# openhumanoids/pronto

Measured on AMD Instinct MI355X. Metric: EKF predict+update steps/sec (batched filters), 15-state, 1000 Hz IMU, higher is better.
Workload: dtype f64

## Files before the change

### pronto_amd/csrc/rbis_coop.hpp

```cpp
#pragma once

#include "rbis_device.hpp"

namespace pb {

template <int NS>
struct Coop {
  static constexpr bool HB = (NS == 21);
  static constexpr int NSC = HB ? 15 : 9;
  static constexpr int NPC = NSC * (NSC + 1) / 2;
  static constexpr int NB_ = HB ? 6 : 0;
  static constexpr bool LL_IN_P = !HB;
  static constexpr int XCH_LLI = 9 + 3 * NSC;
  static constexpr int NXCH = 9 + 3 * NSC + (LL_IN_P ? 1 : 0);
  PB_HD static constexpr int fullc(int s) { return core_full(s); }
  PB_HD static constexpr int fullp(int p) { return passive_full(p); }
};

struct ProcBlocks {
  double a_mw[3];
  double a_g[3];
  double a_mv[3];
  double A_R[9];
  double A_RV[9];
// ... 344 lines not shown
      for (int j = 0; j <= i; j++)
        S2[pk(i, j)] = Pc[pk(CORR::sub[i], CORR::sub[j])] + (i == j ? (cin.upd ? cin.rd[i] : 1.0) : (cin.upd ? cin.ro[i * (i - 1) / 2 + j] : 0.0));
    ldlt<M>(S2, d2);
    double quad2 = 0.0, det2 = 1.0;
#pragma unroll
    for (int kk = 0; kk < M; kk++) {
      double s2 = r2[kk];
#pragma unroll
      for (int j = 0; j < kk; j++) s2 -= S2[pk(kk, j)] * y2[j];
      y2[kk] = cin.upd ? s2 : 0.0;
      id2[kk] = cin.upd ? 1.0 / d2[kk] : 0.0;
      yd2[kk] = y2[kk] * id2[kk];
      det2 *= d2[kk];
      quad2 += s2 * s2 * id2[kk];
    }
    const double lli2 = -log(det2) - quad2;
    if constexpr (C::LL_IN_P) xw(CX::X2_LLI, lli2);
    else if (cin.upd) ll += lli2;
    constexpr bool W2_LDS = C::HB;
    double W2[W2_LDS ? 1 : NSC][M];
    double dfull2[NS];
#pragma unroll
    for (int i = 0; i < NS; i++) dfull2[i] = 0.0;
#pragma unroll
    for (int i = 1; i < M; i++)
#pragma unroll
      for (int j = 0; j < i; j++) xw(CX::X2_L + i * (i - 1) / 2 + j, S2[pk(i, j)]);
#pragma unroll
    for (int kk = 0; kk < M; kk++) { xw(CX::X2_ID + kk, id2[kk]); xw(CX::X2_YD + kk, yd2[kk]); }
#pragma unroll
    for (int i = 0; i < NSC; i++) {
      double w2[M], dxs = 0.0;
#pragma unroll
      for (int kk = 0; kk < M; kk++) {
        double s2 = Pc[pk(i, CORR::sub[kk])];
#pragma unroll
        for (int j = 0; j < kk; j++) s2 -= w2[j] * S2[pk(kk, j)];
        w2[kk] = s2;
        xw(CX::X2_W + M * i + kk, s2);
        dxs = (kk == 0) ? s2 * yd2[0] : fma(s2, yd2[kk], dxs);
        if constexpr (!W2_LDS) W2[i][kk] = s2;
      }
      dfull2[C::fullc(i)] = dxs;
    }
    sync();
#pragma unroll
    for (int i = 0; i < NSC; i++) {
      if constexpr (W2_LDS) reload_fence();
      double wd2[M];
#pragma unroll
      for (int kk = 0; kk < M; kk++) wd2[kk] = (W2_LDS ? xr(CX::X2_W + M * i + kk) : W2[i][kk]) * id2[kk];
#pragma unroll
      for (int j = 0; j <= i; j++) {
        double acc = Pc[pk(i, j)];
#pragma unroll
        for (int kk = 0; kk < M; kk++) acc = fma(-wd2[kk], W2_LDS ? xr(CX::X2_W + M * j + kk) : W2[j][kk], acc);
        st(L::OFF_P + pk(C::fullc(i), C::fullc(j)), acc);
      }
    }
    if constexpr (SIX == 2) {
#pragma unroll
      for (int i = 0; i < NS; i++) dfull2[i] += dfull[i];
      if (upd1 || cin.upd) add_delta<NS>(x, q, dfull2, k.chi_tol);
    } else {
      if (cin.upd) add_delta<NS>(x, q, dfull2, k.chi_tol);
    }
  }
  if constexpr (!UPDATE && CORR::M == 0) {
#pragma unroll
    for (int i = 0; i < NSC; i++)
#pragma unroll
      for (int j = 0; j <= i; j++) st(L::OFF_P + pk(C::fullc(i), C::fullc(j)), Pc[pk(i, j)]);
    sync();
  }
#pragma unroll
  for (int i = 0; i < 9; i++) st(L::OFF_VEC + C::fullc(i), x[C::fullc(i)]);
#pragma unroll
  for (int i = 0; i < 4; i++) st(L::OFF_QUAT + i, q[i]);
  if constexpr (!C::LL_IN_P) st(L::OFF_LL, ll);
#pragma unroll
  for (int i = 9; i < NSC; i++) st(L::OFF_VEC + C::fullc(i), x[C::fullc(i)]);
}

template <int NS, bool UPDATE, class CORR = NoCorr, bool PREDICT = true, int SIX = 0, class LD, class ST, class XW, class XR, class SYNC,
          class SP = NoPredStore>
PB_HD void coop_role_passive_x(LD ld, ST st, XW xw, XR xr, SYNC sync, const StepInputs &in, const Consts &k,
                               const CorrInputs &cin = CorrInputs(), const SixIn &six = SixIn(), SP sp = SP())
{
  static_assert(!SP::on || (PREDICT && UPDATE && CORR::M == 0 && SIX == 0), "the predicted rows: the plain fused step only");
  static_assert(SIX != 1 || (UPDATE && PREDICT && CORR::M == 0), "SIX == 1 rides on a predict + velocity update");
  using L = Lay<NS>;
  using C = Coop<NS>;
  double x[NS], q[4] = { 1.0, 0.0, 0.0, 0.0 };
#pragma unroll
  for (int i = 0; i < NS; i++) x[i] = 0.0;
  if constexpr (PREDICT) {
#pragma unroll
    for (int i = 0; i < NS; i++) x[i] = ld(L::OFF_VEC + i);
#pragma unroll
    for (int i = 0; i < 4; i++) q[i] = ld(L::OFF_QUAT + i);
  } else {
#pragma unroll
    for (int i = 0; i < 6; i++) x[C::fullp(i)] = ld(L::OFF_VEC + C::fullp(i));
  }
  constexpr int NSB = C::HB ? 5 : 3;
  double X[NSB][2][9];
#pragma unroll
  for (int sb = 0; sb < NSB; sb++)
#pragma unroll
    for (int J = 0; J < 2; J++)
#pragma unroll
      for (int r = 0; r < 3; r++)
#pragma unroll
        for (int c = 0; c < 3; c++) X[sb][J][3 * r + c] = ld(L::OFF_P + pk(C::fullc(3 * sb + r), C::fullp(3 * J + c)));
  double Ppp[21];
#pragma unroll
  for (int i = 0; i < 6; i++)
#pragma unroll
    for (int j = 0; j <= i; j++) Ppp[pk(i, j)] = ld(L::OFF_P + pk(C::fullp(i), C::fullp(j)));
  double ll = 0.0;
  if constexpr (C::LL_IN_P) ll = ld(L::OFF_LL);

  double xp[6];
  if constexpr (!PREDICT) {
#pragma unroll
    for (int i = 0; i < 6; i++) xp[i] = x[C::fullp(i)];
  }
  if constexpr (PREDICT) {
  ProcBlocks f;
  make_proc_blocks<NS>(x, q, in.dt, k, f);
#pragma unroll
  for (int J = 0; J < 2; J++) {
    double nD[9], nV[9], nC[9];
#pragma unroll
    for (int i = 0; i < 9; i++) { nD[i] = X[2][J][i]; nV[i] = X[0][J][i]; nC[i] = X[1][J][i]; }
    mat_mul_acc(f.A_R, X[0][J], nD);
    mat_mul_acc(f.A_RV, X[1][J], nD);
    hat_mul_acc(f.a_mw, X[0][J], nV);
    hat_mul_acc(f.a_g, X[1][J], nV);
    hat_mul_acc(f.a_mw, X[1][J], nC);
    if constexpr (C::HB) {
      hat_mul_acc(f.a_mv, X[3][J], nV);
#pragma unroll
      for (int i = 0; i < 9; i++) {
        nV[i] -= in.dt * X[4][J][i];
        nC[i] -= in.dt * X[3][J][i];
      }
    }
#pragma unroll
    for (int i = 0; i < 9; i++) { X[2][J][i] = nD[i]; X[0][J][i] = nV[i]; X[1][J][i] = nC[i]; }
  }
#pragma unroll
  for (int r = 0; r < 3; r++)
#pragma unroll
    for (int c = 0; c <= r; c++) {
      Ppp[pk(r, c)] = (r == c) ? in.qg : 0.0;
      Ppp[pk(3 + r, 3 + c)] = (r == c) ? in.qa : 0.0;
    }
#pragma unroll
  for (int i = 0; i < 3; i++) {
    xp[i] = in.gyro[i] - (C::HB ? x[15 + i] : 0.0);
    xp[3 + i] = in.accel[i] - (C::HB ? x[18 + i] : 0.0);
  }
  }
  if constexpr (SP::on) {
#pragma unroll
    for (int J = 0; J < 2; J++)
#pragma unroll
      for (int sb = 0; sb < NSB; sb++)
#pragma unroll
        for (int r = 0; r < 3; r++)
#pragma unroll
          for (int c = 0; c < 3; c++) sp(L::OFF_P + pk(C::fullc(3 * sb + r), C::fullp(3 * J + c)), X[sb][J][3 * r + c]);
#pragma unroll
    for (int i = 0; i < 6; i++)
#pragma unroll
      for (int j = 0; j <= i; j++) sp(L::OFF_P + pk(C::fullp(i), C::fullp(j)), Ppp[pk(i, j)]);
    if constexpr (C::LL_IN_P) sp(L::OFF_LL, ll);
#pragma unroll
    for (int i = 0; i < 6; i++) sp(L::OFF_VEC + C::fullp(i), xp[i]);
  }

  if constexpr (SIX == 1) {
    using CX = CoopX<NS, CORR>;
    const double idw = six.on ? 1.0 / (in.qg + six.r) : 0.0;
    double ydw[3], quad = 0.0;
#pragma unroll
    for (int kk = 0; kk < 3; kk++) {
      const double res = six.on ? six.z[kk] - xp[kk] : 0.0;
      ydw[kk] = res * idw;
      quad = fma(res, ydw[kk], quad);
    }
    const double dw = in.qg + six.r;
    const double lliw = six.on ? -log(dw * dw * dw) - quad : 0.0;
    xw(CX::X6_ID, idw);
#pragma unroll
    for (int kk = 0; kk < 3; kk++) xw(CX::X6_YD + kk, ydw[kk]);
    if constexpr (!C::LL_IN_P) xw(CX::X6_LLI, lliw);
    else ll += lliw;
#pragma unroll
    for (int sb = 0; sb < NSB; sb++)
#pragma unroll
      for (int r = 0; r < 3; r++)
#pragma unroll
        for (int kk = 0; kk < 3; kk++) xw(CX::X6_A + 3 * (3 * sb + r) + kk, X[sb][0][3 * r + kk]);
    sync();
    const double keep = fma(-in.qg, idw, 1.0);
#pragma unroll
    for (int sb = 0; sb < NSB; sb++)
#pragma unroll
      for (int r = 0; r < 3; r++) {
        const double ad[3] = { X[sb][0][3 * r] * idw, X[sb][0][3 * r + 1] * idw, X[sb][0][3 * r + 2] * idw };
#pragma unroll
        for (int c = 0; c < 3; c++) {
          X[sb][1][3 * r + c] = fma(-ad[2], Ppp[pk(3 + c, 2)], fma(-ad[1], Ppp[pk(3 + c, 1)], fma(-ad[0], Ppp[pk(3 + c, 0)], X[sb][1][3 * r + c])));
          X[sb][0][3 * r + c] *= keep;
        }
      }
#pragma unroll
    for (int r = 0; r < 3; r++) {
      const double ad[3] = { Ppp[pk(3 + r, 0)] * idw, Ppp[pk(3 + r, 1)] * idw, Ppp[pk(3 + r, 2)] * idw };
      xp[3 + r] += fma(Ppp[pk(3 + r, 2)], ydw[2], fma(Ppp[pk(3 + r, 1)], ydw[1], Ppp[pk(3 + r, 0)] * ydw[0]));
#pragma unroll
      for (int c = 0; c <= r; c++)
        Ppp[pk(3 + r, 3 + c)] = fma(-ad[2], Ppp[pk(3 + c, 2)], fma(-ad[1], Ppp[pk(3 + c, 1)], fma(-ad[0], Ppp[pk(3 + c, 0)], Ppp[pk(3 + r, 3 + c)])));
    }
#pragma unroll
    for (int r = 0; r < 3; r++) {
#pragma unroll
      for (int c = 0; c < 3; c++) Ppp[pk(3 + r, c)] *= keep;
      Ppp[pk(r, r)] = in.qg * keep;
      xp[r] = fma(in.qg, ydw[r], xp[r]);
    }
  }
  if constexpr (!UPDATE && CORR::M == 0) sync();
  if constexpr (UPDATE) {
    sync();
    const double L10 = xr(0), L20 = xr(1), L21 = xr(2);
    double id[3], yd[3];
#pragma unroll
    for (int kk = 0; kk < 3; kk++) { id[kk] = xr(3 + kk); yd[kk] = xr(6 + kk); }
    double Wp[6][3];
#pragma unroll
    for (int pi = 0; pi < 6; pi++) {
      const double c0 = X[0][pi / 3][0 * 3 + pi % 3], c1 = X[0][pi / 3][1 * 3 + pi % 3], c2 = X[0][pi / 3][2 * 3 + pi % 3];
      Wp[pi][0] = c0;
      Wp[pi][1] = c1 - Wp[pi][0] * L10;
      Wp[pi][2] = c2 - Wp[pi][0] * L20 - Wp[pi][1] * L21;
      xp[pi] += fma(Wp[pi][2], yd[2], fma(Wp[pi][1], yd[1], Wp[pi][0] * yd[0]));
    }
    if constexpr (C::LL_IN_P) {
      const double lli = xr(C::XCH_LLI);
      if (in.upd) ll += lli;
    }
#pragma unroll
    for (int J = 0; J < 2; J++)
#pragma unroll
      for (int sb = 0; sb < NSB; sb++)
#pragma unroll
        for (int r = 0; r < 3; r++) {
          double wd[3];
#pragma unroll
          for (int kk = 0; kk < 3; kk++) wd[kk] = xr(9 + 3 * (3 * sb + r) + kk) * id[kk];
#pragma unroll
          for (int c = 0; c < 3; c++) {
            double acc = X[sb][J][3 * r + c];
#pragma unroll
            for (int kk = 0; kk < 3; kk++) acc = fma(-wd[kk], Wp[3 * J + c][kk], acc);
            if constexpr (CORR::M == 0) st(L::OFF_P + pk(C::fullc(3 * sb + r), C::fullp(3 * J + c)), acc);
            else X[sb][J][3 * r + c] = acc;
          }
        }
#pragma unroll
    for (int i = 0; i < 6; i++) {
      double wd[3];
#pragma unroll
      for (int kk = 0; kk < 3; kk++) wd[kk] = Wp[i][kk] * id[kk];
#pragma unroll
      for (int j = 0; j <= i; j++) {
        double acc = Ppp[pk(i, j)];
#pragma unroll
        for (int kk = 0; kk < 3; kk++) acc = fma(-wd[kk], Wp[j][kk], acc);
        if constexpr (CORR::M == 0) st(L::OFF_P + pk(C::fullp(i), C::fullp(j)), acc);
        else Ppp[pk(i, j)] = acc;
      }
    }
  }
  if constexpr (CORR::M > 0) {
    constexpr int M = CORR::M;
    using CX = CoopX<NS, CORR>;
    sync();
    double id2[M], yd2[M], L2[M * (M - 1) / 2 + 1];
#pragma unroll
    for (int i = 0; i < M * (M - 1) / 2; i++) L2[i] = xr(CX::X2_L + i);
#pragma unroll
    for (int kk = 0; kk < M; kk++) { id2[kk] = xr(CX::X2_ID + kk); yd2[kk] = xr(CX::X2_YD + kk); }
    if constexpr (C::LL_IN_P) {
      const double lli2 = xr(CX::X2_LLI);
      if (cin.upd) ll += lli2;
    }
    double W2p[6][M];
#pragma unroll
    for (int pi = 0; pi < 6; pi++) {
      double dxs = 0.0;
#pragma unroll
      for (int kk = 0; kk < M; kk++) {
        double s2 = X[CORR::sub[kk] / 3][pi / 3][(CORR::sub[kk] % 3) * 3 + pi % 3];
#pragma unroll
        for (int j = 0; j < kk; j++) s2 -= W2p[pi][j] * L2[kk * (kk - 1) / 2 + j];
        W2p[pi][kk] = s2;
        dxs = (kk == 0) ? s2 * yd2[0] : fma(s2, yd2[kk], dxs);
      }
      xp[pi] += dxs;
    }
#pragma unroll
    for (int J = 0; J < 2; J++)
#pragma unroll
      for (int sb = 0; sb < NSB; sb++)
#pragma unroll
        for (int r = 0; r < 3; r++) {
          double wd2[M];
#pragma unroll
          for (int kk = 0; kk < M; kk++) wd2[kk] = xr(CX::X2_W + M * (3 * sb + r) + kk) * id2[kk];
#pragma unroll
          for (int c = 0; c < 3; c++) {
            double acc = X[sb][J][3 * r + c];
#pragma unroll
            for (int kk = 0; kk < M; kk++) acc = fma(-wd2[kk], W2p[3 * J + c][kk], acc);
            st(L::OFF_P + pk(C::fullc(3 * sb + r), C::fullp(3 * J + c)), acc);
          }
        }
#pragma unroll
    for (int i = 0; i < 6; i++) {
      double wd2[M];
#pragma unroll
      for (int kk = 0; kk < M; kk++) wd2[kk] = W2p[i][kk] * id2[kk];
#pragma unroll
      for (int j = 0; j <= i; j++) {
        double acc = Ppp[pk(i, j)];
#pragma unroll
        for (int kk = 0; kk < M; kk++) acc = fma(-wd2[kk], W2p[j][kk], acc);
        st(L::OFF_P + pk(C::fullp(i), C::fullp(j)), acc);
      }
    }
  }
  if constexpr (!UPDATE && CORR::M == 0) {
#pragma unroll
    for (int J = 0; J < 2; J++)
#pragma unroll
      for (int sb = 0; sb < NSB; sb++)
#pragma unroll
        for (int r = 0; r < 3; r++)
#pragma unroll
          for (int c = 0; c < 3; c++) st(L::OFF_P + pk(C::fullc(3 * sb + r), C::fullp(3 * J + c)), X[sb][J][3 * r + c]);
#pragma unroll
    for (int i = 0; i < 6; i++)
#pragma unroll
      for (int j = 0; j <= i; j++) st(L::OFF_P + pk(C::fullp(i), C::fullp(j)), Ppp[pk(i, j)]);
  }
  if constexpr (C::LL_IN_P) st(L::OFF_LL, ll);
#pragma unroll
  for (int i = 0; i < 6; i++) st(L::OFF_VEC + C::fullp(i), xp[i]);
}
template <int NS, bool UPDATE, class CORR = NoCorr, bool PREDICT = true, class LD, class ST, class XR, class SYNC, class SP = NoPredStore>
PB_HD void coop_role_passive(LD ld, ST st, XR xr, SYNC sync, const StepInputs &in, const Consts &k,
                             const CorrInputs &cin = CorrInputs(), SP sp = SP())
{
  coop_role_passive_x<NS, UPDATE, CORR, PREDICT, 0>(ld, st, [](int, double) {}, xr, sync, in, k, cin, SixIn(), sp);
}

}
```

### pronto_amd/csrc/rbis_device.hpp

```cpp
#pragma once

#include <cmath>
#include <type_traits>
#include <utility>

#if defined(__HIPCC__)
#include <hip/hip_runtime.h>
#define PB_HD __host__ __device__ __forceinline__
#else
#define PB_HD inline
#endif

namespace pb {

template <int NS>
struct Lay {
  static constexpr int NB = NS / 3;
  static constexpr int NP = NS * (NS + 1) / 2;
  static constexpr int OFF_VEC = 0;
  static constexpr int OFF_QUAT = NS;
  static constexpr int OFF_LL = NS + 4;
  static constexpr int OFF_P = NS + 5;
  static constexpr int NC = NS + 5 + NP;
};

PB_HD constexpr int pk(int i, int j) { return i >= j ? i * (i + 1) / 2 + j : j * (j + 1) / 2 + i; }

PB_HD void reload_fence() { asm volatile("" ::: "memory"); }

PB_HD constexpr int pk_row(int p)
{
  int i = 0;
  while ((i + 1) * (i + 2) / 2 <= p) i++;
  return i;
}
PB_HD constexpr int pk_col(int p) { return p - pk_row(p) * (pk_row(p) + 1) / 2; }

template <class Fn, int... I>
PB_HD void static_for_impl(Fn &&fn, std::integer_sequence<int, I...>)
{
  (fn(std::integral_constant<int, I>{}), ...);
}
template <int N, class Fn>
PB_HD void static_for(Fn &&fn)
{
  static_for_impl(fn, std::make_integer_sequence<int, N>{});
}

PB_HD constexpr int core_full(int s) { return s < 9 ? 3 + s : 15 + (s - 9); }
PB_HD constexpr int passive_full(int p) { return p < 3 ? p : 12 + (p - 3); }

template <int NS>
struct Slots {
  using L = Lay<NS>;
  static constexpr bool HB = (NS == 21);
  static constexpr int NSC = HB ? 15 : 9;
  static constexpr int NSB = HB ? 5 : 3;
  static constexpr int NROW = (L::NC + 1) / 2, NSLOT = 2 * NROW;
  static constexpr int TILE = 64;
  static constexpr long TILE_DOUBLES = (long) NSLOT * TILE;
  static constexpr unsigned TILE_BYTES = (unsigned) (NSLOT * TILE * 8);
  struct Tab {
    short slot_of[L::NC];
    short comp_of[NSLOT];
    signed char role2[NSLOT];
    bool split2[NROW];
    int ncore;
    int nq[4];
  };
  static constexpr Tab make()
  {
    Tab t{};
    int s = 0, role = 0;
    auto put = [&](int c) { t.slot_of[c] = (short) s; t.role2[s] = (signed char) role; t.comp_of[s++] = (short) c; };
    if (!HB) {
      for (int i = 0; i < 9; i++) put(L::OFF_VEC + 3 + i);
      for (int i = 0; i < 4; i++) put(L::OFF_QUAT + i);
      for (int i = 0; i < 9; i++)
        for (int j = 0; j <= i; j++) put(L::OFF_P + pk(core_full(i), core_full(j)));
      t.ncore = s;
      t.nq[0] = t.nq[1] = s;
      role = 1;
      for (int J = 0; J < 2; J++)
        for (int i = 0; i < NSC; i++)
          for (int cc = 0; cc < 3; cc++) put(L::OFF_P + pk(core_full(i), passive_full(3 * J + cc)));
      for (int i = 0; i < 6; i++)
        for (int j = 0; j <= i; j++) put(L::OFF_P + pk(passive_full(i), passive_full(j)));
      put(L::OFF_LL);
      for (int i = 0; i < 6; i++) put(L::OFF_VEC + passive_full(i));
      t.nq[2] = s;
    } else {
      for (int i = 0; i < 9; i++)
        for (int j = 0; j <= i; j++) put(L::OFF_P + pk(core_full(i), core_full(j)));
      put(L::OFF_LL);
      t.nq[0] = s;
      for (int i = 9; i < NSC; i++)
        for (int j = 0; j <= i; j++) put(L::OFF_P + pk(core_full(i), core_full(j)));
      for (int i = 0; i < 6; i++) put(L::OFF_VEC + 15 + i);
      role = 1;
      for (int i = 0; i < 3; i++) put(L::OFF_VEC + passive_full(i));
      t.nq[1] = s;
      t.ncore = s;
      for (int i = 0; i < NSC; i++)
        for (int cc = 0; cc < 3; cc++) put(L::OFF_P + pk(core_full(i), passive_full(cc)));
      for (int i = 0; i < 3; i++)
        for (int j = 0; j <= i; j++) put(L::OFF_P + pk(passive_full(i), passive_full(j)));
      role = 0;
      for (int i = 0; i < 9; i++) put(L::OFF_VEC + 3 + i);
      for (int i = 0; i < 4; i++) put(L::OFF_QUAT + i);
      t.nq[2] = s;
      role = 1;
      for (int i = 0; i < NSC; i++)
        for (int cc = 0; cc < 3; cc++) put(L::OFF_P + pk(core_full(i), passive_full(3 + cc)));
      for (int i = 3; i < 6; i++)
        for (int j = 0; j <= i; j++) put(L::OFF_P + pk(passive_full(i), passive_full(j)));
      for (int i = 3; i < 6; i++) put(L::OFF_VEC + passive_full(i));
    }
    while (s < NSLOT) { t.role2[s] = (signed char) role; t.comp_of[s++] = -1; }
    t.nq[3] = s;
    for (int r = 0; r < NROW; r++) t.split2[r] = t.role2[2 * r] != t.role2[2 * r + 1];
    return t;
  }
  static constexpr Tab T = make();
  static_assert(T.nq[0] % 2 == 0 && T.nq[1] % 2 == 0 && T.nq[2] % 2 == 0, "every wave must own whole rows");
  static constexpr int ROW_SPLIT = T.ncore / 2;
  static constexpr int QROW[5] = { 0, T.nq[0] / 2, T.nq[1] / 2, T.nq[2] / 2, T.nq[3] / 2 };
  PB_HD static constexpr int slot(int comp) { return T.slot_of[comp]; }
  PB_HD static long eidx(int comp, long b)
  {
    const int sl = T.slot_of[comp];
    return (b >> 6) * TILE_DOUBLES + (long) (sl >> 1) * (2 * TILE) + (b & 63) * 2 + (sl & 1);
  }
  PB_HD static long eidx_slot(int sl, long b) { return (b >> 6) * TILE_DOUBLES + (long) (sl >> 1) * (2 * TILE) + (b & 63) * 2 + (sl & 1); }
};

enum { BW = 0, BV = 1, BCHI = 2, BPOS = 3, BACC = 4, BBG = 5, BBA = 6 };

struct Consts {
  double g;
  double chi_tol;
  const double *qblk = nullptr;
  int xcd_remap = 0;
  int half_tiles = 0;
};

PB_HD void quat_mul(const double (&a)[4], const double (&b)[4], double (&o)[4])
{
  const double w = a[0] * b[0] - a[1] * b[1] - a[2] * b[2] - a[3] * b[3];
  const double x = a[0] * b[1] + a[1] * b[0] + a[2] * b[3] - a[3] * b[2];
  const double y = a[0] * b[2] + a[2] * b[0] + a[3] * b[1] - a[1] * b[3];
  const double z = a[0] * b[3] + a[3] * b[0] + a[1] * b[2] - a[2] * b[1];
  o[0] = w; o[1] = x; o[2] = y; o[3] = z;
}

PB_HD void quat_to_rot(const double (&q)[4], double (&R)[9])
{
  const double w = q[0], x = q[1], y = q[2], z = q[3];
  const double tx = 2 * x, ty = 2 * y, tz = 2 * z;
  const double twx = tx * w, twy = ty * w, twz = tz * w;
  const double txx = tx * x, txy = ty * x, txz = tz * x;
  const double tyy = ty * y, tyz = tz * y, tzz = tz * z;
  R[0] = 1 - (tyy + tzz); R[1] = txy - twz;       R[2] = txz + twy;
  R[3] = txy + twz;       R[4] = 1 - (txx + tzz); R[5] = tyz - twx;
  R[6] = txz - twy;       R[7] = tyz + twx;       R[8] = 1 - (txx + tyy);
}

PB_HD void sincos_joint(double x, double &s, double &c)
{
  const double kf = rint(x * 6.36619772367581382433e-01);
  double r = fma(-kf, 1.57079632673412561417e+00, x);
  r = fma(-kf, 6.07710050650619224932e-11, r);
  const double z = r * r;
  double ps = 1.58969099521155010221e-10;
  ps = fma(ps, z, -2.50507602534068634195e-08);
  ps = fma(ps, z, 2.75573137070700676789e-06);
  ps = fma(ps, z, -1.98412698298579493134e-04);
  ps = fma(ps, z, 8.33333333332248946124e-03);
  ps = fma(ps, z, -1.66666666666666324348e-01);
  const double sn = fma(r * z, ps, r);
  double pc = -1.13596475577881948265e-11;
  pc = fma(pc, z, 2.08757232129817482790e-09);
  pc = fma(pc, z, -2.75573143513906633035e-07);
  pc = fma(pc, z, 2.48015872894767294178e-05);
  pc = fma(pc, z, -1.38888888888741095749e-03);
  pc = fma(pc, z, 4.16666666666666019037e-02);
  const double cs = fma(z * z, pc, fma(-0.5, z, 1.0));
  const int k = (int) kf & 3;
  const double a = (k & 1) ? cs : sn, b = (k & 1) ? sn : cs;
  s = (k & 2) ? -a : a;
  c = ((k + 1) & 2) ? -b : b;
}

PB_HD void fold_chi(double (&chi)[3], double (&q)[4], double tol)
{
  const double n = sqrt(chi[0] * chi[0] + chi[1] * chi[1] + chi[2] * chi[2]);
  if (n > tol) {
    double s, c;
    sincos_joint(0.5 * n, s, c);
    const double f = s / n;
    const double dq[4] = { c, f * chi[0], f * chi[1], f * chi[2] };
    double o[4];
    quat_mul(q, dq, o);
    q[0] = o[0]; q[1] = o[1]; q[2] = o[2]; q[3] = o[3];
    chi[0] = chi[1] = chi[2] = 0.0;
  }
}

template <int NS>
// ... 385 lines not shown
```

### pronto_amd/csrc/rbis_kernels.hpp

```cpp
#pragma once

#include <hip/hip_runtime.h>
#include <stdint.h>

#include "../../include/pronto_batch.h"
#include "rbis_coop.hpp"
#include "rbis_quad.hpp"
#include "rbis_device.hpp"

#define PB_STEP_BLOCK 64

namespace pb {

typedef unsigned v2u __attribute__((ext_vector_type(2)));
typedef unsigned v4u __attribute__((ext_vector_type(4)));
typedef double d2_t __attribute__((ext_vector_type(2)));
typedef __amdgpu_buffer_rsrc_t rsrc_t;

__device__ __forceinline__ rsrc_t mkbuf(const void *p, unsigned bytes)
{
  return __builtin_amdgcn_make_buffer_rsrc(const_cast<void *>(p), 0, bytes, 0x00020000);
}
template <int AUX = 0>
__device__ __forceinline__ double ldg(rsrc_t r, unsigned soff, unsigned voff)
// ... 69 lines not shown
#pragma unroll
    for (int r = R0; r < R1; r++) fetch(r);
  }
  __device__ __forceinline__ double ld(int comp)
  {
    const int s = S::T.slot_of[comp];
    fetch(s >> 1);
    return (s & 1) ? cache[s >> 1].y : cache[s >> 1].x;
  }
  __device__ __forceinline__ void st(int comp, double v)
  {
    const int s = S::T.slot_of[comp];
    if (TWO_ROLE && S::T.split2[s >> 1]) {
      stg<SA>(ro, (unsigned) (s >> 1) * 1024u + (unsigned) (s & 1) * 8u, vo, v);
      return;
    }
    outv[s] = v;
    have[s] = true;
    if (have[s ^ 1]) {
      const d2_t o = { outv[s & ~1], outv[s | 1] };
      stg2<SA>(ro, (unsigned) (s >> 1) * 1024u, vo, o);
    }
  }
  __device__ __forceinline__ double ld_slot_rt(int slot) const
  {
    return ldg(rs, (unsigned) (slot >> 1) * 1024u + (unsigned) (slot & 1) * 8u, vo);
  }
};

template <int NS>
__device__ __forceinline__ int slot_rt(int comp)
{
  return Slots<NS>::T.slot_of[comp];
}
__device__ __forceinline__ int pk_rt(int i, int j) { return i >= j ? i * (i + 1) / 2 + j : j * (j + 1) / 2 + i; }

struct IdxVel {
  static constexpr Idx<3> value = { { 3, 4, 5 } };
};

template <int NS, bool UPDATE, int MH = MH_DEFAULT>
__global__ __launch_bounds__(PB_STEP_BLOCK, 1) void k_step(const double *st, double *sto, int B,
                                                const double *__restrict__ imu, const double *__restrict__ lo,
                                                const uint8_t *__restrict__ mask, double qg, double qa, double qbg,
                                                double qba, Consts k, StepBcast bc)
{
  using L = Lay<NS>;
  const unsigned tile = xcd_workgroup(k);
  const unsigned b = tile * 64u + threadIdx.x;
  if (b >= (unsigned) B) return;
  const unsigned bo = b * 8u, B8 = (unsigned) B * 8u;
  TileIO<NS, MemHint<MH>::LA, MemHint<MH>::SA> io(st, sto, tile, threadIdx.x);
  const rsrc_t ri = mkbuf(imu, 7u * B8);
  const rsrc_t rl = mkbuf(lo, UPDATE ? 6u * B8 : 0u);
  double gyro[3], accel[3], dt, z[3], rd[3];
  bool upd = false;
  if constexpr (UPDATE) upd = (mask == nullptr) || (mask[b] != 0);
  if (bc.on & 1) {
#pragma unroll
    for (int i = 0; i < 3; i++) { gyro[i] = bc.imu[i]; accel[i] = bc.imu[3 + i]; }
    dt = bc.imu[6];
  } else {
#pragma unroll
    for (int i = 0; i < 3; i++) {
      gyro[i] = ldg(ri, i * B8, bo);
      accel[i] = ldg(ri, (3 + i) * B8, bo);
    }
    dt = ldg(ri, 6u * B8, bo);
  }
  if (bc.on & 2) {
#pragma unroll
    for (int i = 0; i < 3; i++) { z[i] = bc.lo[i]; rd[i] = bc.lo[3 + i]; }
  } else {
#pragma unroll
    for (int i = 0; i < 3; i++) {
      z[i] = UPDATE ? ldg(rl, i * B8, bo) : 0.0;
      rd[i] = UPDATE ? ldg(rl, (3 + i) * B8, bo) : 1.0;
    }
  }
  if (k.qblk != nullptr) {
    const rsrc_t rq = mkbuf(k.qblk, 4u * B8);
    qg = ldg(rq, 0u, bo); qa = ldg(rq, B8, bo); qbg = ldg(rq, 2u * B8, bo); qba = ldg(rq, 3u * B8, bo);
  }
  io.template need<0, Slots<NS>::NROW>();
  double x[NS], q[4], ll, P[L::NP];
#pragma unroll
  for (int i = 0; i < NS; i++) x[i] = io.ld(L::OFF_VEC + i);
#pragma unroll
  for (int i = 0; i < 4; i++) q[i] = io.ld(L::OFF_QUAT + i);
  ll = io.ld(L::OFF_LL);
#pragma unroll
  for (int i = 0; i < L::NP; i++) P[i] = io.ld(L::OFF_P + i);
  imu_process_step<NS>(x, q, P, gyro, accel, dt, qg, qa, qbg, qba, k);
  if constexpr (UPDATE) {
    double resid[3], S[6];
#pragma unroll
    for (int i = 0; i < 3; i++) resid[i] = upd ? z[i] - x[3 + i] : 0.0;
#pragma unroll
    for (int i = 0; i < 3; i++)
#pragma unroll
      for (int j = 0; j <= i; j++)
        S[pk(i, j)] = P[pk(3 + i, 3 + j)] + (i == j ? (upd ? rd[i] : 1.0) : 0.0);
    measurement_update<NS, 3>(x, q, P, ll, resid, S, IdxVel{}, k, [&io](int pi, double v) { io.st(L::OFF_P + pi, v); }, upd);
  } else {
#pragma unroll
    for (int i = 0; i < L::NP; i++) io.st(L::OFF_P + i, P[i]);
  }
#pragma unroll
  for (int i = 0; i < NS; i++) io.st(L::OFF_VEC + i, x[i]);
#pragma unroll
  for (int i = 0; i < 4; i++) io.st(L::OFF_QUAT + i, q[i]);
  io.st(L::OFF_LL, ll);
}

template <int NS>
__global__ __launch_bounds__(64, 1) void k_replay_fused(double *__restrict__ st, int B, int T,
                                                        const double *__restrict__ imu, const double *__restrict__ lo,
                                                        const uint8_t *__restrict__ mask, double qg, double qa, double qbg,
                                                        double qba, Consts k)
{
  using L = Lay<NS>;
  const unsigned b = blockIdx.x * blockDim.x + threadIdx.x;
  if (b >= (unsigned) B) return;
  const unsigned bo = b * 8u, B8 = (unsigned) B * 8u;
  TileIO<NS, 0, 0> io(st, st, blockIdx.x, threadIdx.x);
  io.template need<0, Slots<NS>::NROW>();
  double x[NS], q[4], ll, P[L::NP];
#pragma unroll
  for (int i = 0; i < NS; i++) x[i] = io.ld(L::OFF_VEC + i);
#pragma unroll
  for (int i = 0; i < 4; i++) q[i] = io.ld(L::OFF_QUAT + i);
  ll = io.ld(L::OFF_LL);
#pragma unroll
  for (int i = 0; i < L::NP; i++) P[i] = io.ld(L::OFF_P + i);
  if (k.qblk != nullptr) {
    const rsrc_t rq = mkbuf(k.qblk, 4u * B8);
    qg = ldg(rq, 0u, bo); qa = ldg(rq, B8, bo); qbg = ldg(rq, 2u * B8, bo); qba = ldg(rq, 3u * B8, bo);
  }
  double in[13];
  bool upd;
  auto fetch = [&](int t, double (&dst)[13], bool &u) {
    const rsrc_t ri = mkbuf(imu + (size_t) t * 7 * B, 7u * B8);
    const rsrc_t rl = mkbuf(lo + (size_t) t * 6 * B, 6u * B8);
#pragma unroll
    for (int i = 0; i < 7; i++) dst[i] = ldg(ri, i * B8, bo);
#pragma unroll
    for (int i = 0; i < 6; i++) dst[7 + i] = ldg(rl, i * B8, bo);
    u = (mask == nullptr) || (mask[(size_t) t * B + b] != 0);
  };
  fetch(0, in, upd);
  for (int t = 0; t < T; t++) {
    if (t > 0) fetch(t, in, upd);
    const double gyro[3] = { in[0], in[1], in[2] }, accel[3] = { in[3], in[4], in[5] };
    imu_process_step<NS>(x, q, P, gyro, accel, in[6], qg, qa, qbg, qba, k);
    double resid[3], S[6];
#pragma unroll
    for (int i = 0; i < 3; i++) resid[i] = upd ? in[7 + i] - x[3 + i] : 0.0;
#pragma unroll
    for (int i = 0; i < 3; i++)
#pragma unroll
      for (int j = 0; j <= i; j++) S[pk(i, j)] = P[pk(3 + i, 3 + j)] + (i == j ? (upd ? in[10 + i] : 1.0) : 0.0);
    measurement_update<NS, 3>(x, q, P, ll, resid, S, IdxVel{}, k, NoSink(), upd);
  }
#pragma unroll
  for (int i = 0; i < L::NP; i++) io.st(L::OFF_P + i, P[i]);
#pragma unroll
  for (int i = 0; i < NS; i++) io.st(L::OFF_VEC + i, x[i]);
// ... 255 lines not shown
  for (int i = 0; i < 4; i++) io.st(L::OFF_QUAT + i, q[i]);
  io.st(L::OFF_LL, ll);
}

template <int NS, bool UPDATE, int MH = MH_DEFAULT, class CORR = NoCorr, bool PREDICT = true>
__global__ __launch_bounds__(128, 1) void k_step_coop(const double *st, double *sto, int B,
                                                      const double *__restrict__ imu, const double *__restrict__ lo,
                                                      const uint8_t *__restrict__ mask, double qg, double qa,
                                                      double qbg, double qba, Consts k, CorrArgs ca, StepBcast bc = StepBcast())
{
  __shared__ double xch[(UPDATE || CORR::M > 0) ? CoopX<NS, CORR>::NXCH : 1][64];
  const int role = __builtin_amdgcn_readfirstlane((int) (threadIdx.x >> 6));
  const unsigned wgi = xcd_workgroup(k);
  const unsigned tile = k.half_tiles ? (wgi >> 1) : wgi;
  const unsigned lane = k.half_tiles ? ((threadIdx.x & 31u) | ((wgi & 1u) << 5)) : (threadIdx.x & 63u);
  const unsigned b = tile * 64u + lane;
  const unsigned bo = b * 8u, B8 = (unsigned) B * 8u;
  TileIO<NS, MemHint<MH>::LA, MemHint<MH>::SA, true> io(st, sto, tile, lane);
  const rsrc_t ri = mkbuf(imu, PREDICT ? 7u * B8 : 0u);
  const rsrc_t rl = mkbuf(lo, UPDATE ? 6u * B8 : 0u);
  StepInputs in;
  if (PREDICT && (bc.on & 1)) {
#pragma unroll
    for (int i = 0; i < 3; i++) { in.gyro[i] = bc.imu[i]; in.accel[i] = bc.imu[3 + i]; }
    in.dt = bc.imu[6];
  } else {
#pragma unroll
    for (int i = 0; i < 3; i++) {
      in.gyro[i] = PREDICT ? ldg(ri, i * B8, bo) : 0.0;
      in.accel[i] = PREDICT ? ldg(ri, (3 + i) * B8, bo) : 0.0;
    }
    in.dt = PREDICT ? ldg(ri, 6u * B8, bo) : 0.0;
  }
  if (PREDICT && (bc.on & 2)) {
#pragma unroll
    for (int i = 0; i < 3; i++) { in.z[i] = bc.lo[i]; in.rd[i] = bc.lo[3 + i]; }
  } else {
#pragma unroll
    for (int i = 0; i < 3; i++) {
      in.z[i] = UPDATE ? ldg(rl, i * B8, bo) : 0.0;
      in.rd[i] = UPDATE ? ldg(rl, (3 + i) * B8, bo) : 1.0;
    }
  }
  in.upd = UPDATE && (b < (unsigned) B) && (mask == nullptr || mask[b] != 0);
  in.qg = qg; in.qa = qa; in.qbg = qbg; in.qba = qba;
  if (PREDICT && k.qblk != nullptr) {
    const rsrc_t rq = mkbuf(k.qblk, 4u * B8);
    in.qg = ldg(rq, 0u, bo); in.qa = ldg(rq, B8, bo); in.qbg = ldg(rq, 2u * B8, bo); in.qba = ldg(rq, 3u * B8, bo);
  }
  CorrInputs cin;
  if constexpr (CORR::M > 0) {
    const rsrc_t rz = mkbuf(ca.z2, (unsigned) CORR::M * B8);
    const rsrc_t rr = mkbuf(ca.r2, ca.r2 ? (unsigned) CORR::M * B8 : 0u);
    const rsrc_t rq2 = mkbuf(ca.qm2, CORR::ORIENT ? 4u * B8 : 0u);
#pragma unroll
    for (int i = 0; i < CORR::M; i++) {
      cin.z[i] = ca.zbc ? ca.zb2[i] : ldg(rz, i * B8, bo);
      cin.rd[i] = ca.r2 ? ldg(rr, i * B8, bo) : ca.rb2[i];
    }
    if (ca.rfull != nullptr) {
      const rsrc_t rf = mkbuf(ca.rfull, (unsigned) (CORR::M * CORR::M) * B8);
#pragma unroll
      for (int i = 0; i < CORR::M; i++) {
        cin.rd[i] = ldg(rf, (unsigned) (i * CORR::M + i) * B8, bo);
#pragma unroll
        for (int j = 0; j < i; j++) cin.ro[i * (i - 1) / 2 + j] = ldg(rf, (unsigned) (j * CORR::M + i) * B8, bo);
      }
    }
#pragma unroll
    for (int i = 0; i < 4; i++) cin.qm[i] = CORR::ORIENT ? (ca.zbc ? ca.qb2[i] : ldg(rq2, i * B8, bo)) : 0.0;
    cin.upd = (b < (unsigned) B) && (ca.mask2 == nullptr || ca.mask2[b] != 0);
    if constexpr (!PREDICT && !UPDATE) {
      if (st == sto && ca.mask2 != nullptr && __ballot(cin.upd) == 0ull) return;
    }
  }
  auto ld = [&io](int comp) { return io.ld(comp); };
  auto stf = [&io](int comp, double v) { io.st(comp, v); };
  auto sync = []() { __syncthreads(); };
  auto xrd = [lane](int s) { return xch[s][lane]; };
  if (role == 0) {
    io.template need<0, Slots<NS>::ROW_SPLIT>();
    coop_role_core<NS, UPDATE, CORR, PREDICT>(ld, stf, [lane](int s, double v) { xch[s][lane] = v; }, xrd, sync, in, k, cin);
  } else {
    io.template need<Slots<NS>::ROW_SPLIT, Slots<NS>::NROW>();
    coop_role_passive<NS, UPDATE, CORR, PREDICT>(ld, stf, xrd, sync, in, k, cin);
  }
}

template <class IO>
struct PredStore {
  static constexpr bool on = true;
  IO *io;
  __device__ __forceinline__ void operator()(int comp, double v) const { io->st(comp, v); }
};

template <int NS, int MH = MH_DEFAULT>
__global__ __launch_bounds__(128, 1) void k_step_coop_pred(const double *st, double *sto, double *pred, int B,
                                                           const double *__restrict__ imu, const double *__restrict__ lo,
                                                           const uint8_t *__restrict__ mask, double qg, double qa,
                                                           double qbg, double qba, Consts k, StepBcast bc)
{
  __shared__ double xch[CoopX<NS, NoCorr>::NXCH][64];
  const int role = __builtin_amdgcn_readfirstlane((int) (threadIdx.x >> 6));
  const unsigned wgi = xcd_workgroup(k);
  const unsigned tile = k.half_tiles ? (wgi >> 1) : wgi;
  const unsigned lane = k.half_tiles ? ((threadIdx.x & 31u) | ((wgi & 1u) << 5)) : (threadIdx.x & 63u);
  const unsigned b = tile * 64u + lane;
  const unsigned bo = b * 8u, B8 = (unsigned) B * 8u;
  using IO = TileIO<NS, MemHint<MH>::LA, MemHint<MH>::SA, true>;
  IO io(st, sto, tile, lane);
  IO po(pred, pred, tile, lane);
  const rsrc_t ri = mkbuf(imu, 7u * B8);
  const rsrc_t rl = mkbuf(lo, 6u * B8);
  StepInputs in;
  if (bc.on & 1) {
#pragma unroll
    for (int i = 0; i < 3; i++) { in.gyro[i] = bc.imu[i]; in.accel[i] = bc.imu[3 + i]; }
    in.dt = bc.imu[6];
  } else {
#pragma unroll
    for (int i = 0; i < 3; i++) { in.gyro[i] = ldg(ri, i * B8, bo); in.accel[i] = ldg(ri, (3 + i) * B8, bo); }
    in.dt = ldg(ri, 6u * B8, bo);
  }
  if (bc.on & 2) {
#pragma unroll
    for (int i = 0; i < 3; i++) { in.z[i] = bc.lo[i]; in.rd[i] = bc.lo[3 + i]; }
  } else {
#pragma unroll
    for (int i = 0; i < 3; i++) { in.z[i] = ldg(rl, i * B8, bo); in.rd[i] = ldg(rl, (3 + i) * B8, bo); }
  }
  in.upd = (b < (unsigned) B) && (mask == nullptr || mask[b] != 0);
  in.qg = qg; in.qa = qa; in.qbg = qbg; in.qba = qba;
  if (k.qblk != nullptr) {
    const rsrc_t rq = mkbuf(k.qblk, 4u * B8);
    in.qg = ldg(rq, 0u, bo); in.qa = ldg(rq, B8, bo); in.qbg = ldg(rq, 2u * B8, bo); in.qba = ldg(rq, 3u * B8, bo);
  }
  auto ld = [&io](int comp) { return io.ld(comp); };
  auto stf = [&io](int comp, double v) { io.st(comp, v); };
  auto sync = []() { __syncthreads(); };
  auto xrd = [lane](int s) { return xch[s][lane]; };
  const PredStore<IO> sp{ &po };
  if (role == 0) {
    io.template need<0, Slots<NS>::ROW_SPLIT>();
    coop_role_core<NS, true, NoCorr, true, false, 0>(ld, stf, [lane](int s, double v) { xch[s][lane] = v; }, xrd, sync, in, k, CorrInputs(), sp);
  } else {
    io.template need<Slots<NS>::ROW_SPLIT, Slots<NS>::NROW>();
    coop_role_passive<NS, true, NoCorr, true>(ld, stf, xrd, sync, in, k, CorrInputs(), sp);
  }
}

template <bool UPDATE, int MH = MH_DEFAULT>
__global__ __launch_bounds__(256, 2) void k_step_quad(const double *st, double *sto, int B,
                                                      const double *__restrict__ imu, const double *__restrict__ lo,
                                                      const uint8_t *__restrict__ mask, double qg, double qa,
                                                      double qbg, double qba, Consts k, StepBcast bc)
{
  using SL = Slots<21>;
  __shared__ double xch[Quad::NXCH][64];
  const int role = __builtin_amdgcn_readfirstlane((int) (threadIdx.x >> 6));
  const unsigned lane = threadIdx.x & 63u;
  const unsigned tile = xcd_workgroup(k);
  const unsigned b = tile * 64u + lane;
  const unsigned bo = b * 8u, B8 = (unsigned) B * 8u;
  TileIO<21, MemHint<MH>::LA, MemHint<MH>::SA> io(st, sto, tile, lane);
  auto inputs = [&](bool meas) {
    const rsrc_t ri = mkbuf(imu, 7u * B8);
    const rsrc_t rl = mkbuf(lo, UPDATE ? 6u * B8 : 0u);
// ... 472 lines not shown
```

Measured before the change: 2.732 billion.

## Reorder passive state slots so predict skips loading dead rows

Reorders the packed state slot table for the 15-state case so the passive components whose prior values are overwritten by predict (the attitude/velocity-noise blocks and their vector entries) sit at the end. Loads then stop at a new ROW_DEAD boundary instead of fetching all rows. Passive-role P updates are kept in registers and written through a shared tail routine in the new order. This cuts global memory reads per filter, but it changes the storage layout and assumes those trailing slots are never needed on input.

Result: slower. 2.670 billion (-2.3%).

```diff
diff --git a/pronto_amd/csrc/rbis_coop.hpp b/pronto_amd/csrc/rbis_coop.hpp
--- a/pronto_amd/csrc/rbis_coop.hpp
+++ b/pronto_amd/csrc/rbis_coop.hpp
@@ -450,6 +450,39 @@
   for (int i = 9; i < NSC; i++) st(L::OFF_VEC + C::fullc(i), x[C::fullc(i)]);
 }
 
+template <int NS, class EMIT>
+PB_HD void passive_tail(EMIT emit, const double (&Ppp)[21], double ll, const double (&xp)[6])
+{
+  using L = Lay<NS>;
+  using C = Coop<NS>;
+  if constexpr (C::HB) {
+#pragma unroll
+    for (int i = 0; i < 6; i++)
+#pragma unroll
+      for (int j = 0; j <= i; j++) emit(L::OFF_P + pk(C::fullp(i), C::fullp(j)), Ppp[pk(i, j)]);
+#pragma unroll
+    for (int i = 0; i < 6; i++) emit(L::OFF_VEC + C::fullp(i), xp[i]);
+  } else {
+#pragma unroll
+    for (int i = 3; i < 6; i++)
+#pragma unroll
+      for (int j = 0; j < 3; j++) emit(L::OFF_P + pk(C::fullp(i), C::fullp(j)), Ppp[pk(i, j)]);
+    emit(L::OFF_LL, ll);
+#pragma unroll
+    for (int i = 0; i < 3; i++) emit(L::OFF_VEC + C::fullp(i), xp[i]);
+#pragma unroll
+    for (int i = 0; i < 3; i++)
+#pragma unroll
+      for (int j = 0; j <= i; j++) emit(L::OFF_P + pk(C::fullp(i), C::fullp(j)), Ppp[pk(i, j)]);
+#pragma unroll
+    for (int i = 3; i < 6; i++)
+#pragma unroll
+      for (int j = 3; j <= i; j++) emit(L::OFF_P + pk(C::fullp(i), C::fullp(j)), Ppp[pk(i, j)]);
+#pragma unroll
+    for (int i = 3; i < 6; i++) emit(L::OFF_VEC + C::fullp(i), xp[i]);
+  }
+}
+
 template <int NS, bool UPDATE, class CORR = NoCorr, bool PREDICT = true, int SIX = 0, class LD, class ST, class XW, class XR, class SYNC,
           class SP = NoPredStore>
 PB_HD void coop_role_passive_x(LD ld, ST st, XW xw, XR xr, SYNC sync, const StepInputs &in, const Consts &k,
@@ -540,13 +573,7 @@
         for (int r = 0; r < 3; r++)
 #pragma unroll
           for (int c = 0; c < 3; c++) sp(L::OFF_P + pk(C::fullc(3 * sb + r), C::fullp(3 * J + c)), X[sb][J][3 * r + c]);
-#pragma unroll
-    for (int i = 0; i < 6; i++)
-#pragma unroll
-      for (int j = 0; j <= i; j++) sp(L::OFF_P + pk(C::fullp(i), C::fullp(j)), Ppp[pk(i, j)]);
-    if constexpr (C::LL_IN_P) sp(L::OFF_LL, ll);
-#pragma unroll
-    for (int i = 0; i < 6; i++) sp(L::OFF_VEC + C::fullp(i), xp[i]);
+    passive_tail<NS>(sp, Ppp, ll, xp);
   }
 
   if constexpr (SIX == 1) {
@@ -649,8 +676,7 @@
         double acc = Ppp[pk(i, j)];
 #pragma unroll
         for (int kk = 0; kk < 3; kk++) acc = fma(-wd[kk], Wp[j][kk], acc);
-        if constexpr (CORR::M == 0) st(L::OFF_P + pk(C::fullp(i), C::fullp(j)), acc);
-        else Ppp[pk(i, j)] = acc;
+        Ppp[pk(i, j)] = acc;
       }
     }
   }
@@ -708,7 +734,7 @@
         double acc = Ppp[pk(i, j)];
 #pragma unroll
         for (int kk = 0; kk < M; kk++) acc = fma(-wd2[kk], W2p[j][kk], acc);
-        st(L::OFF_P + pk(C::fullp(i), C::fullp(j)), acc);
+        Ppp[pk(i, j)] = acc;
       }
     }
   }
@@ -721,14 +747,8 @@
         for (int r = 0; r < 3; r++)
 #pragma unroll
           for (int c = 0; c < 3; c++) st(L::OFF_P + pk(C::fullc(3 * sb + r), C::fullp(3 * J + c)), X[sb][J][3 * r + c]);
-#pragma unroll
-    for (int i = 0; i < 6; i++)
-#pragma unroll
-      for (int j = 0; j <= i; j++) st(L::OFF_P + pk(C::fullp(i), C::fullp(j)), Ppp[pk(i, j)]);
-  }
-  if constexpr (C::LL_IN_P) st(L::OFF_LL, ll);
-#pragma unroll
-  for (int i = 0; i < 6; i++) st(L::OFF_VEC + C::fullp(i), xp[i]);
+  }
+  passive_tail<NS>(st, Ppp, ll, xp);
 }
 template <int NS, bool UPDATE, class CORR = NoCorr, bool PREDICT = true, class LD, class ST, class XR, class SYNC, class SP = NoPredStore>
 PB_HD void coop_role_passive(LD ld, ST st, XR xr, SYNC sync, const StepInputs &in, const Consts &k,
diff --git a/pronto_amd/csrc/rbis_device.hpp b/pronto_amd/csrc/rbis_device.hpp
--- a/pronto_amd/csrc/rbis_device.hpp
+++ b/pronto_amd/csrc/rbis_device.hpp
@@ -66,6 +66,7 @@
     signed char role2[NSLOT];
     bool split2[NROW];
     int ncore;
+    int nlive;
     int nq[4];
   };
   static constexpr Tab make()
@@ -84,10 +85,16 @@
       for (int J = 0; J < 2; J++)
         for (int i = 0; i < NSC; i++)
           for (int cc = 0; cc < 3; cc++) put(L::OFF_P + pk(core_full(i), passive_full(3 * J + cc)));
-      for (int i = 0; i < 6; i++)
+      for (int i = 3; i < 6; i++)
+        for (int j = 0; j < 3; j++) put(L::OFF_P + pk(passive_full(i), passive_full(j)));
+      put(L::OFF_LL);
+      for (int i = 0; i < 3; i++) put(L::OFF_VEC + passive_full(i));
+      t.nlive = s;
+      for (int i = 0; i < 3; i++)
         for (int j = 0; j <= i; j++) put(L::OFF_P + pk(passive_full(i), passive_full(j)));
-      put(L::OFF_LL);
-      for (int i = 0; i < 6; i++) put(L::OFF_VEC + passive_full(i));
+      for (int i = 3; i < 6; i++)
+        for (int j = 3; j <= i; j++) put(L::OFF_P + pk(passive_full(i), passive_full(j)));
+      for (int i = 3; i < 6; i++) put(L::OFF_VEC + passive_full(i));
       t.nq[2] = s;
     } else {
       for (int i = 0; i < 9; i++)
@@ -124,6 +131,7 @@
   static constexpr Tab T = make();
   static_assert(T.nq[0] % 2 == 0 && T.nq[1] % 2 == 0 && T.nq[2] % 2 == 0, "every wave must own whole rows");
   static constexpr int ROW_SPLIT = T.ncore / 2;
+  static constexpr int ROW_DEAD = HB ? NROW : (T.nlive + 1) / 2;
   static constexpr int QROW[5] = { 0, T.nq[0] / 2, T.nq[1] / 2, T.nq[2] / 2, T.nq[3] / 2 };
   PB_HD static constexpr int slot(int comp) { return T.slot_of[comp]; }
   PB_HD static long eidx(int comp, long b)
diff --git a/pronto_amd/csrc/rbis_kernels.hpp b/pronto_amd/csrc/rbis_kernels.hpp
--- a/pronto_amd/csrc/rbis_kernels.hpp
+++ b/pronto_amd/csrc/rbis_kernels.hpp
@@ -175,7 +175,7 @@
     const rsrc_t rq = mkbuf(k.qblk, 4u * B8);
     qg = ldg(rq, 0u, bo); qa = ldg(rq, B8, bo); qbg = ldg(rq, 2u * B8, bo); qba = ldg(rq, 3u * B8, bo);
   }
-  io.template need<0, Slots<NS>::NROW>();
+  io.template need<0, Slots<NS>::ROW_DEAD>();
   double x[NS], q[4], ll, P[L::NP];
 #pragma unroll
   for (int i = 0; i < NS; i++) x[i] = io.ld(L::OFF_VEC + i);
@@ -597,7 +597,7 @@
     io.template need<0, Slots<NS>::ROW_SPLIT>();
     coop_role_core<NS, UPDATE, CORR, PREDICT>(ld, stf, [lane](int s, double v) { xch[s][lane] = v; }, xrd, sync, in, k, cin);
   } else {
-    io.template need<Slots<NS>::ROW_SPLIT, Slots<NS>::NROW>();
+    io.template need<Slots<NS>::ROW_SPLIT, PREDICT ? Slots<NS>::ROW_DEAD : Slots<NS>::NROW>();
     coop_role_passive<NS, UPDATE, CORR, PREDICT>(ld, stf, xrd, sync, in, k, cin);
   }
 }
```
